# 115dkk/Impulcifer-pip313

Measured on AMD Instinct MI355X. Metric: impulse responses/sec (sweep deconv+FIR), 7.1×2-ear @48kHz, 1/2/4/8 GPU, higher is better.
Workload: dtype f32

## Files before the change

### impulcifer-pip313_amd/csrc/conv_kernels.hip.h

```cpp
#pragma once
#include "fft_regs.hip.h"

namespace imp {

constexpr int kN2 = 4096;
constexpr int kLogN2 = 12;
constexpr int kRowPad = 272;
#ifndef IMP_AB_PREFETCH
#define IMP_AB_PREFETCH 8
#endif
constexpr int kAbPrefetch = IMP_AB_PREFETCH;

struct Twiddles {
  const cf* __restrict__ full;
  const cf* __restrict__ hi;
  const cf* __restrict__ t1;
  const cf* __restrict__ t2;
  const cf* __restrict__ t4;
};

__device__ __forceinline__ void xcd_work_item(int nchan, int& tile, int& chan) {
  const int xcd = blockIdx.x & 7;
  const int slot = blockIdx.x >> 3;
  const int tl = slot / nchan;
// ... 818 lines not shown
#pragma unroll
  for (int j = 0; j < 16; ++j) bstore_cf<IMP_AUX_ROWS_ST>(v[j], r_row, vo8, j * 256 * 8);
}

struct FirBlockArgs {
  const float4* __restrict__ ab;
  long long ab_chan_stride;
  float* __restrict__ out;
  long long out_stride;
  long long out_start, out_len;
  int kp;
  int valid;
  int blocks;
  int first_block;
  int nchan;
};

constexpr int kFirBlockPoints = 4 * kN2;
constexpr size_t kFirBlockLds = sizeof(cf) * 4 * 16 * kRowPad;

template <class L, class = void> struct LoadHasDeviceLen { static constexpr bool value = false; };
template <class L> struct LoadHasDeviceLen<L, decltype((void)L::kDeviceLen)> { static constexpr bool value = true; };

template <class Load>
__global__ __launch_bounds__(1024, 4) void fir_block_kernel(Load ld, FirBlockArgs a, Twiddles tw) {
  extern __shared__ __attribute__((aligned(16))) char smem_raw[];
  cf* lds = reinterpret_cast<cf*>(smem_raw);
  const int xcd = blockIdx.x & 7, slot = blockIdx.x >> 3;
  const int chan = (slot / a.blocks) * 8 + xcd, blk = a.first_block + slot % a.blocks;
  if (chan >= a.nchan) return;
  long long out_len = a.out_len;
  int filt = chan;
  if constexpr (LoadHasDeviceLen<Load>::value) {
    out_len = ld.out_len(chan);
    filt = ld.filter_of(chan);
    if ((long long)blk * a.valid - a.out_start >= out_len) return;
  }
  const int tid = threadIdx.x;
  const int pairq = __builtin_amdgcn_readfirstlane(tid >> 9);
  const int half = __builtin_amdgcn_readfirstlane((tid >> 8) & 1);
  const int t = tid & 255;
  const int k1 = pairq + 2 * half;
  const int s0 = blk * a.valid - a.kp;
  const __amdgpu_buffer_rsrc_t r_full = make_rsrc(tw.full, 4u * kN2 * 8u);
  const auto row = ld.open(chan);

  cf v[16];
#pragma unroll
  for (int h = 0; h < 2; ++h) {
    cf x[2][4], w[2][3];
#pragma unroll
    for (int c = 0; c < 2; ++c) {
      const int n2 = tid + 1024 * (2 * h + c);
#pragma unroll
      for (int n1 = 0; n1 < 4; ++n1) x[c][n1] = row.pair_at(s0 + 2 * (n1 * kN2 + n2));
#pragma unroll
      for (int k = 1; k < 4; ++k) w[c][k - 1] = bload_cf(r_full, (unsigned)(k * kN2 + n2) * 8u, 0u);
    }
#pragma unroll
    for (int c = 0; c < 2; ++c) {
      const int n2 = tid + 1024 * (2 * h + c);
#pragma unroll
      for (int n1 = 0; n1 < 4; ++n1) x[c][n1] = row.finish(x[c][n1], s0 + 2 * (n1 * kN2 + n2));
      bfly4<-1>(x[c][0], x[c][1], x[c][2], x[c][3]);
      lds[n2] = x[c][0];
#pragma unroll
      for (int k = 1; k < 4; ++k) lds[k * kN2 + n2] = cmul(x[c][k], w[c][k - 1]);
    }
// ... 18 lines not shown
    cf w0 = lds[n2], w1 = lds[kN2 + n2], w2 = lds[2 * kN2 + n2], w3 = lds[3 * kN2 + n2];
    w1 = cmulc(w1, bload_cf(r_full, (unsigned)(kN2 + n2) * 8u, 0u));
    w2 = cmulc(w2, bload_cf(r_full, (unsigned)(2 * kN2 + n2) * 8u, 0u));
    w3 = cmulc(w3, bload_cf(r_full, (unsigned)(3 * kN2 + n2) * 8u, 0u));
    bfly4<+1>(w0, w1, w2, w3);
    const cf y[4] = {w0, w1, w2, w3};
#pragma unroll
    for (int n1 = 0; n1 < 4; ++n1) {
      const int pos = 2 * (n1 * kN2 + n2);
      if (pos < a.kp) continue;
      const unsigned off = (unsigned)(o0 + pos) * 4u;
      if (a.out_start & 1) {
        unsigned off_im = off + 4u;
        asm volatile("" : "+v"(off_im));
        __builtin_amdgcn_raw_buffer_store_b32(__float_as_uint(y[n1].x), r_out, off, 0u, 0);
        __builtin_amdgcn_raw_buffer_store_b32(__float_as_uint(y[n1].y), r_out, off_im, 0u, 0);
      } else {
        bstore_cf<kStreamAux>(y[n1], r_out, off, 0u);
      }
    }
  }
}

}
```

### impulcifer-pip313_amd/csrc/impulse_hip.hip

```cpp
#include <hip/hip_runtime.h>

#include <algorithm>
#include <cmath>
#include <complex>
#include <cstdarg>
#include <cstdio>
#include <cstdlib>
#include <cstring>
#include <map>
#include <mutex>
#include <new>
#include <string>
#include <vector>

#include "internal.h"
#include "conv_kernels.hip.h"
#include "ir_kernels.hip.h"
#include "decay_kernels.hip.h"
#include "slice_kernels.hip.h"

static thread_local std::string g_last_error;

int imp_fail(int code, const char* fmt, ...) {
  char buf[1024];
  va_list ap;
  va_start(ap, fmt);
  vsnprintf(buf, sizeof(buf), fmt, ap);
  va_end(ap);
  g_last_error = buf;
  return code;
}

int ctx_bind(imp_ctx* ctx) {
// ... 994 lines not shown
  if (!p->timing) return IMP_OK;
  if (slot == 0) p->group_timed = (p->group_counter++ % p->timing) == 0;
  if (!p->group_timed) return IMP_OK;
  if (p->timed >= kMaxTimed) {
    int rc = plan_collect_timing(p);
    if (rc) return rc;
  }
  const size_t need = (size_t)(4 * (p->timed + 1));
  while (p->events.size() < need) {
    hipEvent_t ev;
    HIP_TRY(hipEventCreate(&ev));
    p->events.push_back(ev);
  }
  HIP_TRY(hipEventRecord(p->events[(size_t)(4 * p->timed + slot)], p->cur_stream));
  if (slot == 3) ++p->timed;
  return IMP_OK;
}

template <class Load>
static int run_group_with(imp_plan* p, Load ld, int64_t nchan, float* d_y, int64_t chan_stride_out,
                          int64_t first_chan, int last_stage);

template <class Load>
static int launch_fir_block(imp_plan* p, Load ld, int64_t nchan, float* d_y, int64_t chan_stride_out, int64_t first_chan) {
  auto kern = imp::fir_block_kernel<Load>;
  int rc = ctx_kernel_lds(p->ctx, reinterpret_cast<const void*>(kern), imp::kFirBlockLds);
  if (rc) return rc;
  const int64_t plane = (int64_t)4 * imp::kN2;
  imp::FirBlockArgs a;
  a.ab = p->ab + (p->n_filters > 1 ? first_chan * plane : 0);
  a.ab_chan_stride = p->n_filters > 1 ? plane : 0;
  a.out = d_y;
  a.out_stride = chan_stride_out;
  a.out_start = p->out_start;
  a.first_block = (int)p->f_first;
  a.out_len = p->out_len;
  a.kp = p->f_kp;
  a.valid = p->f_valid;
  a.blocks = (int)p->f_blocks;
  a.nchan = (int)nchan;
  imp::Twiddles tw{p->tw.full, p->tw.hi, p->ctx->tw_t1, p->ctx->tw_t2, p->ctx->tw_t4};
  dim3 grid((unsigned)((nchan + 7) / 8 * 8 * p->f_blocks)), block(1024);
  hipLaunchKernelGGL(kern, grid, block, imp::kFirBlockLds, p->cur_stream, ld, a, tw);
  HIP_TRY(hipGetLastError());
  return IMP_OK;
}

template <class Load>
static int run_group_pair(imp_plan* p, Load ld, int64_t nchan, float* d_y, int64_t chan_stride_out, int last_stage) {
  int rc;
  const int64_t lane_channels = p->ws_channels / p->lanes;
  const int lane = (p->lanes > 1) ? (int)(p->group_counter_lane++ % p->lanes) : 0;
  p->cur_stream = lane ? p->ctx->side_streams[(size_t)(lane - 1)] : p->ctx->stream;
  p->cur_ws = p->ws + (int64_t)lane * (lane_channels / 2) * p->N1 * imp::kN2;
  if (nchan < 1 || nchan > lane_channels || (lane_channels & 1))
    return fail(IMP_ERR_INVALID, "launch group of %lld channels exceeds the workspace lane (%lld, whole pairs)",
                (long long)nchan, (long long)lane_channels);
  const int64_t npairs = (nchan + 1) / 2;
  if ((double)(chan_stride_out + p->out_len) * 4.0 >= 4294967296.0)
    return fail(IMP_ERR_INVALID, "chan_stride_out %lld: a pair's two output rows must lie within 4 GiB", (long long)chan_stride_out);
  imp::StoreWorkspace stw{p->cur_ws, p->N1};
  if ((rc = timing_event(p, 0))) return rc;
  if ((rc = launch_cols_any<-1>(p, npairs, ld, stw))) return rc;
  if ((rc = timing_event(p, 1))) return rc;
  if (last_stage < 1) return IMP_OK;
  if ((rc = launch_rows_single(p, npairs))) return rc;
  if ((rc = timing_event(p, 2))) return rc;
// ... 373 lines not shown
  return rc;
}

struct imp_chain {
  imp_ctx* ctx = nullptr;
  imp_ctx* tail_ctx = nullptr;
  imp_plan* deconv = nullptr;
  imp_plan* fir = nullptr;
  int64_t B = 0, n = 0, head = 0, fade_in = 0, fade_out = 0, pitch_ir = 0;
  double peak_height = 0.12589;
  int lanes = 1;
  int sets = 1;
  int64_t calls = 0;
  int tiles = 0;
  int64_t chunks = 0;
  std::vector<float*> d_ir;
  std::vector<unsigned*> d_tile;
  std::vector<imp::RowPeak*> d_res;
  std::vector<hipEvent_t> k1_done;
  std::vector<hipEvent_t> ir_free;
  std::vector<char> ir_busy;
  int64_t* d_meta = nullptr;
  double* d_win = nullptr;
};

struct ChainLock {
  std::unique_lock<std::recursive_mutex> a, b;
  ChainLock(imp_ctx* x, imp_ctx* y) {
    if (x == y) {
      a = std::unique_lock<std::recursive_mutex>(x->mu);
    } else {
      imp_ctx* lo = x < y ? x : y;
      imp_ctx* hi = x < y ? y : x;
      a = std::unique_lock<std::recursive_mutex>(lo->mu);
      b = std::unique_lock<std::recursive_mutex>(hi->mu);
    }
  }
};

extern "C" void imp_chain_destroy(imp_chain* c) {
  if (!c) return;
  ChainLock lk(c->ctx, c->tail_ctx);
  (void)hipSetDevice(c->ctx->device);
  (void)plan_sync_lanes(c->deconv);
  (void)hipStreamSynchronize(c->tail_ctx->stream);
  for (auto p : c->d_ir) (void)hipFree(p);
// ... 28 lines not shown
  if (fir->n_filters > 1 && B > fir->n_filters) return fail(IMP_ERR_INVALID, "imp_chain_create: fewer FIRs than channels");
  if (n > deconv->out_len || head < 0 || fade_in < 0 || fade_out < 0 || fade_in > n || fade_out > n)
    return fail(IMP_ERR_INVALID, "imp_chain_create: crop of %lld samples with fades %lld / %lld does not fit", (long long)n,
                (long long)fade_in, (long long)fade_out);
  if ((deconv->paired ? deconv->N1 / 2 : deconv->N1) > imp::kMaxPlanRows)
    return fail(IMP_ERR_UNSUPPORTED, "imp_chain_create: deconvolution plan of %d rows", deconv->N1);
  int rc = ctx_bind(deconv->ctx);
  if (rc) return rc;
  imp_chain* c = new (std::nothrow) imp_chain();
  if (!c) return fail(IMP_ERR_ALLOC, "out of host memory");
  c->ctx = deconv->ctx;
  c->tail_ctx = fir->ctx;
  c->deconv = deconv;
  c->fir = fir;
  c->B = B;
  c->n = n;
  c->head = head;
  c->fade_in = fade_in;
  c->fade_out = fade_out;
  c->peak_height = peak_height;
  c->lanes = deconv->lanes;
  c->sets = deconv->ctx == fir->ctx ? 1 : c->lanes + 1;
  c->pitch_ir = (deconv->out_len + 63) / 64 * 64;
  std::vector<int64_t> meta((size_t)(2 * B));
  for (int64_t b = 0; b < B; ++b) {
    meta[(size_t)b] = b * c->pitch_ir;
    meta[(size_t)(B + b)] = deconv->out_len;
  }
  c->tiles = plan_col_tiles(deconv);
  c->chunks = deconv->paired ? deconv->N1 / 2 : deconv->N1;
  const size_t chunk_bytes = (size_t)(B * c->chunks) * sizeof(unsigned);
  bool ok = hipMalloc((void**)&c->d_meta, (size_t)(2 * B) * sizeof(int64_t)) == hipSuccess &&
            hipMemcpy(c->d_meta, meta.data(), meta.size() * sizeof(int64_t), hipMemcpyHostToDevice) == hipSuccess &&
            hipMalloc((void**)&c->d_win, (size_t)std::max<int64_t>(fade_in + fade_out, 1) * sizeof(double)) == hipSuccess;
  if (ok && fade_in + fade_out > 0) {
    hipLaunchKernelGGL(imp::fade_table_kernel, dim3((unsigned)((fade_in + fade_out + 255) / 256)), dim3(256), 0, deconv->ctx->stream,
                       c->d_win, (long long)fade_in, (long long)fade_out);
    ok = hipGetLastError() == hipSuccess && hipStreamSynchronize(deconv->ctx->stream) == hipSuccess;
  }
  for (int l = 0; l < c->sets && ok; ++l) {
    float* ir = nullptr;
    unsigned* tile = nullptr;
    imp::RowPeak* res = nullptr;
    hipEvent_t e1 = nullptr, e2 = nullptr;
    ok = hipMalloc((void**)&ir, (size_t)(B * c->pitch_ir) * sizeof(float)) == hipSuccess;
    if (ir) c->d_ir.push_back(ir);
// ... 20 lines not shown
                                        float* d_out, int64_t chan_stride_out, long long* d_peaks_out) {
  if (!c || !d_x || !d_out) return fail(IMP_ERR_INVALID, "imp_chain_execute_device: null argument");
  ChainLock lk(c->ctx, c->tail_ctx);
  if (chan_stride_out < c->fir->out_len)
    return fail(IMP_ERR_INVALID, "chan_stride_out %lld < out_len %lld", (long long)chan_stride_out, (long long)c->fir->out_len);
  if (c->deconv->lanes != c->lanes || c->fir->lanes != 1)
    return fail(IMP_ERR_INVALID, "imp_chain_execute_device: a plan's overlap setting changed since the chain was made");
  int rc = ctx_bind(c->ctx);
  if (rc) return rc;
  const int lane = c->lanes > 1 ? (int)(c->deconv->group_counter_lane % c->lanes) : 0;
  const int l = (int)(c->calls++ % c->sets);
  hipStream_t lane_stream = lane ? c->ctx->side_streams[(size_t)(lane - 1)] : c->ctx->stream;
  hipStream_t tail = c->tail_ctx->stream;
  if (c->ir_busy[(size_t)l] && tail != lane_stream) HIP_TRY(hipStreamWaitEvent(lane_stream, c->ir_free[(size_t)l], 0));
  c->deconv->tile_max = c->d_tile[(size_t)l];
  rc = imp_conv_execute_device(c->deconv, d_x, c->B, chan_stride_in, elem_stride_in, c->d_ir[(size_t)l], c->pitch_ir);
  c->deconv->tile_max = nullptr;
  if (rc) return rc;
  if (c->deconv->cur_stream != lane_stream) return fail(IMP_ERR_HIP, "imp_chain_execute_device: lane bookkeeping out of step");
  if (tail != lane_stream) {
    HIP_TRY(hipEventRecord(c->k1_done[(size_t)l], lane_stream));
    HIP_TRY(hipStreamWaitEvent(tail, c->k1_done[(size_t)l], 0));
  }
  hipLaunchKernelGGL(imp::row_first_peak_chunked_kernel, dim3((unsigned)c->B), dim3(imp::kPeakThreads), 0, tail, c->d_ir[(size_t)l],
                     c->d_meta, c->d_meta + c->B, c->deconv->out_start, (const unsigned*)c->d_tile[(size_t)l], c->tiles,
                     (const unsigned*)nullptr, c->chunks, c->d_res[(size_t)l], c->peak_height, d_peaks_out);
  HIP_TRY(hipGetLastError());
  imp::LoadCropAtPeak ld{c->d_ir[(size_t)l], c->pitch_ir, c->deconv->out_len, c->d_res[(size_t)l], c->n, c->head, c->fade_in, c->fade_out,
                         c->d_win};
  if ((rc = run_group_with(c->fir, ld, c->B, d_out, chan_stride_out, 0, 2))) return rc;
  if (tail != lane_stream) {
    HIP_TRY(hipEventRecord(c->ir_free[(size_t)l], tail));
    c->ir_busy[(size_t)l] = 1;
  }
  return IMP_OK;
}

struct imp_segset {
  imp_ctx* ctx = nullptr;
  int64_t B = 0;
  double* e = nullptr;
  int64_t* off = nullptr;
  int64_t* len = nullptr;
  std::vector<int64_t> h_len;
  void* qbuf = nullptr;
  size_t qcap = 0;
  void* keep_a = nullptr;
  void* keep_b = nullptr;
  std::vector<int64_t> keep_host;
};

extern "C" void imp_segset_destroy(imp_segset* s) {
  if (!s) return;
// ... 667 lines not shown
```

### impulcifer-pip313_amd/csrc/ir_kernels.hip.h

```cpp
#pragma once
#include <hip/hip_runtime.h>
#include <stdint.h>

#include "conv_kernels.hip.h"

namespace imp {

struct RowPeak {
  unsigned int maxabs_bits;
  unsigned int pad;
  unsigned long long first_peak;
  unsigned long long first_max;
};

constexpr int kPeakChunk = 8192;
#ifdef IMP_PEAK_DIAG
#define IMP_PEAK_T(k) do { if (threadIdx.x == 0 && blockIdx.x == 0) peak_ts[k] = clock64(); } while (0)
#else
#define IMP_PEAK_T(k) do { } while (0)
#endif
constexpr int kPeakThreads = 1024;
constexpr int kMaxPlanRows = 256;

__device__ __forceinline__ int64_t peak_chunks(int64_t n, int64_t shift) {
// ... 7 lines not shown
  __syncthreads();
  if ((threadIdx.x & 63) == 0) wm[threadIdx.x >> 6] = m;
  __syncthreads();
  float r = wm[0];
#pragma unroll
  for (int k = 1; k < NW; ++k) r = fmaxf(r, wm[k]);
  return r;
}

template <int NW>
__device__ __forceinline__ unsigned long long block_min_u64(unsigned long long v, unsigned long long* wm ) {
#pragma unroll
  for (int s = 32; s > 0; s >>= 1) {
    const unsigned long long o = __shfl_xor(v, s, 64);
    v = o < v ? o : v;
  }
  __syncthreads();
  if ((threadIdx.x & 63) == 0) wm[threadIdx.x >> 6] = v;
  __syncthreads();
  unsigned long long r = wm[0];
#pragma unroll
  for (int k = 1; k < NW; ++k) r = wm[k] < r ? wm[k] : r;
  return r;
}

__global__ __launch_bounds__(256) void row_chunk_max_kernel(const float* __restrict__ x, const int64_t* __restrict__ off,
                                                            const int64_t* __restrict__ len, int64_t shift,
                                                            unsigned* __restrict__ chunk_max, int64_t pitch) {
  const int b = blockIdx.y;
  const int64_t n = len[b], c = blockIdx.x;
  if (c >= peak_chunks(n, shift)) return;
  const int64_t lo = c * kPeakChunk - shift > 0 ? c * kPeakChunk - shift : 0;
  const int64_t hi = (c + 1) * kPeakChunk - shift < n ? (c + 1) * kPeakChunk - shift : n;
  const float* row = x + off[b];
  float m = 0.f;
  int64_t i = lo + threadIdx.x;
  for (; i + 7 * 256 < hi; i += 8 * 256) {
    float v[8];
#pragma unroll
    for (int k = 0; k < 8; ++k) v[k] = row[i + k * 256];
#pragma unroll
    for (int k = 0; k < 8; ++k) m = fmaxf(m, fabsf(v[k]));
  }
  for (; i < hi; i += 256) m = fmaxf(m, fabsf(row[i]));
  __shared__ __attribute__((aligned(16))) float wm[4];
  m = block_max_f32<4>(m, wm);
  if (threadIdx.x == 0) chunk_max[(int64_t)b * pitch + c] = __float_as_uint(m);
}

__global__ __launch_bounds__(kPeakThreads) void row_first_peak_chunked_kernel(
    const float* __restrict__ x, const int64_t* __restrict__ off, const int64_t* __restrict__ len, int64_t shift,
    const unsigned* __restrict__ tile_max, int tiles, const unsigned* __restrict__ chunk_max, int64_t pitch,
    RowPeak* __restrict__ res, double height, long long* __restrict__ peaks_out) {
  const int b = blockIdx.x, tid = threadIdx.x;
#ifdef IMP_PEAK_DIAG
  long long peak_ts[8] = {0, 0, 0, 0, 0, 0, 0, 0};
#endif
  IMP_PEAK_T(0);
  const int64_t n = len[b];
  const float* row = x + off[b];
  const int64_t nch = peak_chunks(n, shift);
  constexpr int NW = kPeakThreads / 64;
  __shared__ __attribute__((aligned(16))) float wmf[NW];
  __shared__ __attribute__((aligned(16))) unsigned long long wmu[NW];
  __shared__ float sx[kPeakChunk + 2];
  constexpr int kLdsChunks = 2048;
  __shared__ unsigned srows[kLdsChunks];
  const unsigned* cm = chunk_max + (int64_t)b * pitch;
  if (tiles > 0) {
    for (int r = tid; r < kMaxPlanRows; r += kPeakThreads) srows[r] = 0u;
    __syncthreads();
    const unsigned* tm = tile_max + (int64_t)b * tiles * pitch;
    const int lane = tid & 63, w = tid >> 6;
    for (int64_t r = lane; r < nch; r += 64) {
      unsigned m = 0u;
#pragma unroll 4
      for (int t = w; t < tiles; t += kPeakThreads / 64) {
        const unsigned v = tm[(int64_t)t * pitch + r];
        m = v > m ? v : m;
      }
      if (m) atomicMax(&srows[r], m);
    }
    __syncthreads();
    cm = srows;
  } else if (nch <= kLdsChunks) {
    for (int64_t c = tid; c < nch; c += kPeakThreads) srows[c] = cm[c];
    __syncthreads();
    cm = srows;
  }
  IMP_PEAK_T(1);
  float mf = 0.f;
  for (int64_t c = tid; c < nch; c += kPeakThreads) mf = fmaxf(mf, __uint_as_float(cm[c]));
  const float maxabs = block_max_f32<NW>(mf, wmf);
  RowPeak out;
  out.maxabs_bits = __float_as_uint(maxabs);
  out.pad = 0u;
  out.first_peak = ~0ull;
  out.first_max = ~0ull;
  if (maxabs >= 1e-20f) {
    __shared__ float s_thr;
    if (tid == 0) {
      const double dmax = (double)maxabs;
      float t = (float)(height * dmax);
      if (!(t >= 0.f)) t = 0.f;
      for (int k = 0; k < 4 && t > 0.f && (double)__uint_as_float(__float_as_uint(t) - 1u) / dmax >= height; ++k)
        t = __uint_as_float(__float_as_uint(t) - 1u);
      for (int k = 0; k < 4 && !((double)t / dmax >= height); ++k) t = __uint_as_float(__float_as_uint(t) + 1u);
      s_thr = t;
    }
    __syncthreads();
    const float thr = s_thr;
    IMP_PEAK_T(2);
    unsigned long long c_q = ~0ull;
    for (int64_t c = tid; c < nch; c += kPeakThreads)
      if (__uint_as_float(cm[c]) >= thr && (unsigned long long)c < c_q) c_q = (unsigned long long)c;
    c_q = block_min_u64<NW>(c_q, wmu);
    constexpr int U = (kPeakChunk + kPeakThreads - 1) / kPeakThreads;
    int64_t lo = 0, hi = 0;
    auto stage = [&](int64_t c) {
      lo = c * kPeakChunk - shift > 0 ? c * kPeakChunk - shift : 0;
      hi = (c + 1) * kPeakChunk - shift < n ? (c + 1) * kPeakChunk - shift : n;
      const int64_t cnt = hi - lo + 2;
      float t[U + 1];
#pragma unroll
      for (int u = 0; u <= U; ++u) {
        const int64_t k = tid + (int64_t)u * kPeakThreads, i = lo - 1 + k;
        t[u] = (k < cnt && i >= 0 && i < n) ? row[i] : 0.f;
      }
      __syncthreads();
#pragma unroll
      for (int u = 0; u <= U; ++u) {
        const int64_t k = tid + (int64_t)u * kPeakThreads;
        if (k < cnt) sx[k] = t[u];
      }
      __syncthreads();
    };
    IMP_PEAK_T(3);
    for (int64_t c = c_q == ~0ull ? nch : (int64_t)c_q; c < nch; ++c) {
      if (!(__uint_as_float(cm[c]) >= thr)) continue;
      stage(c);
      IMP_PEAK_T(4);
      float xs[U];
#pragma unroll
      for (int u = 0; u < U; ++u) {
        const int64_t i = lo + tid + (int64_t)u * kPeakThreads;
        xs[u] = i < hi ? sx[i - lo + 1] : 0.f;
      }
      unsigned long long best = ~0ull;
#pragma unroll
      for (int u = 0; u < U; ++u) {
        const int64_t i = lo + tid + (int64_t)u * kPeakThreads;
        const float xi = xs[u];
        if (best != ~0ull || !(fabsf(xi) >= thr) || i >= hi || i == 0 || i >= n - 1) continue;
        const float xm = sx[i - lo];
        const bool up = xm < xi, dn = xm > xi;
        if (!up && !dn) continue;
        if (!((up ? xi : -xi) >= thr)) continue;
        int64_t j = i;
        while (j + 1 < n && (j + 1 <= hi ? sx[j + 1 - lo + 1] : row[j + 1]) == xi) ++j;
        if (j + 1 >= n) continue;
        const float xn = j + 1 <= hi ? sx[j + 1 - lo + 1] : row[j + 1];
        if (up ? (xn < xi) : (xn > xi)) best = (unsigned long long)((i + j) / 2);
      }
      best = block_min_u64<NW>(best, wmu);
      if (best != ~0ull) {
        out.first_peak = best;
        break;
      }
    }
    IMP_PEAK_T(5);
    if (out.first_peak == ~0ull) {
      unsigned long long c_max = ~0ull;
      for (int64_t c = tid; c < nch; c += kPeakThreads)
        if (__uint_as_float(cm[c]) == maxabs && (unsigned long long)c < c_max) c_max = (unsigned long long)c;
      c_max = block_min_u64<NW>(c_max, wmu);
      stage((int64_t)c_max);
      unsigned long long best = ~0ull;
      for (int64_t i = lo + tid; i < hi; i += kPeakThreads)
        if (fabsf(sx[i - lo + 1]) == maxabs) {
          best = (unsigned long long)i;
          break;
        }
      out.first_max = block_min_u64<NW>(best, wmu);
    }
  }
  IMP_PEAK_T(6);
#ifdef IMP_PEAK_DIAG
  if (tid == 0 && b == 0)
    printf("peak phases (clk): entry->fold %lld, max+thr %lld, cq %lld, stage %lld, search %lld, fallback %lld\n", peak_ts[1] - peak_ts[0],
           peak_ts[2] - peak_ts[1], peak_ts[3] - peak_ts[2], peak_ts[4] - peak_ts[3], peak_ts[5] - peak_ts[4], peak_ts[6] - peak_ts[5]);
#endif
  if (tid == 0) {
    res[b] = out;
    if (peaks_out) {
      long long pk;
      if (n == 0 || !(maxabs >= 1e-20f)) pk = 0;
      else pk = (long long)(out.first_peak != ~0ull ? out.first_peak : out.first_max);
      peaks_out[b] = pk;
    }
  }
}

__device__ __forceinline__ double hann_sym_fwd(int64_t i, int64_t N) {
  if (N <= 1) return 1.0;
  return 0.5 - 0.5 * cospi(2.0 * (double)i / (double)(N - 1));
}


__device__ __forceinline__ unsigned* crop_max_lds() {
  __shared__ unsigned rows[kMaxPlanRows];
  return rows;
}

struct StoreRealCropMax {
  StoreRealCrop crop;
  unsigned* __restrict__ tile_max;
  __device__ __forceinline__ __amdgpu_buffer_rsrc_t bind(int b) const { return crop.bind(b); }
  __device__ __forceinline__ void begin(int tid, int threads) const {
    unsigned* rows = crop_max_lds();
    for (int r = tid; r < kMaxPlanRows; r += threads) rows[r] = 0u;
    __syncthreads();
  }
// ... 61 lines not shown
    for (int r = tid; r < chunks; r += threads) out[r] = rl[r];
    if (2 * p + 1 < crop.nchan) {
      out += (long long)tiles * chunks;
      for (int r = tid; r < chunks; r += threads) out[r] = rr[r];
    }
  }
};

struct LoadCropAtPeak {
  const float* __restrict__ base;
  long long chan_stride;
  long long row_len;
  const RowPeak* __restrict__ res;
  long long n, head, fade_in, fade_out;
  const double* __restrict__ win;
  __host__ __device__ LoadCropAtPeak shifted(long long, long long) const { return *this; }
  static __device__ __forceinline__ float shaped(float x, long long i, long long n, long long fade_in, long long fade_out,
                                                 const double* __restrict__ win) {
    double g = 1.0;
    if (i < fade_in) g *= win[i];
    if (fade_out > 0 && i >= n - fade_out && i < n) g *= win[fade_in + (i - (n - fade_out))];
    return (float)((double)x * g);
  }
  __device__ __forceinline__ long long crop_start(int b) const {
    const RowPeak rp = res[b];
    long long pk;
    if (row_len == 0 || !(__uint_as_float(rp.maxabs_bits) >= 1e-20f)) pk = 0;
    else pk = (long long)(rp.first_peak != ~0ull ? rp.first_peak : rp.first_max);
    long long start = pk - head;
    if (start > row_len - n) start = row_len - n;
    if (start < 0) start = 0;
    return start;
  }
  struct Row {
    __amdgpu_buffer_rsrc_t r;
    int n, fade_in, fade_out;
    const double* __restrict__ win;
    __device__ __forceinline__ cf pair_at(int s) const { return bload_cf<0>(r, (unsigned)s * 4u, 0u); }
    __device__ __forceinline__ cf finish(cf v, int s) const {
      if ((unsigned)s < (unsigned)n && (s < fade_in || s + 1 >= n - fade_out)) {
        v.x = shaped(v.x, s, n, fade_in, fade_out, win);
        v.y = shaped(v.y, s + 1, n, fade_in, fade_out, win);
      }
      return v;
    }
  };
  __device__ __forceinline__ Row open(int b) const {
    const long long start = crop_start(b), avail = row_len - start;
    return Row{make_rsrc(base + (long long)b * chan_stride + start, (unsigned)(avail < n ? avail : n) * 4u), (int)n, (int)fade_in,
               (int)fade_out, win};
  }
  template <int STEP, int F>
  __device__ __forceinline__ void column(int b, unsigned e0, cf (&v)[F]) const {
    const long long start = crop_start(b), avail = row_len - start;
    const __amdgpu_buffer_rsrc_t r = make_rsrc(base + (long long)b * chan_stride + start, (unsigned)(avail < n ? avail : n) * 4u);
#pragma unroll
    for (int j = 0; j < F; ++j) {
      const u32x2 x = __builtin_amdgcn_raw_buffer_load_b64(r, e0 * 8u, (unsigned)(j * STEP) * 8u, 0);
      v[j] = make_float2(__uint_as_float(x.x), __uint_as_float(x.y));
      const long long i = 2ll * ((long long)e0 + (long long)j * STEP);
      if (i < n && (i < fade_in || i + 1 >= n - fade_out)) {
        v[j].x = shaped(v[j].x, i, n, fade_in, fade_out, win);
        v[j].y = shaped(v[j].y, i + 1, n, fade_in, fade_out, win);
      }
    }
  }
};

__global__ __launch_bounds__(256) void fade_table_kernel(double* __restrict__ win, long long fade_in, long long fade_out) {
  const long long i = (long long)blockIdx.x * blockDim.x + threadIdx.x;
  if (i < fade_in) win[i] = hann_sym_fwd(i, 2 * fade_in);
  else if (i < fade_in + fade_out) win[i] = hann_sym_fwd(fade_out + (i - fade_in), 2 * fade_out);
}

struct WindowParams {
  float gain;
  int64_t fade_in;
  int64_t fade_out;
  int64_t decay_start;
  int64_t decay_half;
  int64_t decay_knee;
  float decay_level_db;
};

__device__ __forceinline__ double hann_sym(int64_t i, int64_t N) {
  if (N <= 1) return 1.0;
  return 0.5 - 0.5 * cospi(2.0 * (double)i / (double)(N - 1));
}
// ... 565 lines not shown
```

Baseline: 299,400.

## Fold first-peak search into FIR block kernel and add 512-thread pairs variant

The separate row_first_peak_chunked_kernel launch is removed from the chain tail. Each FIR block kernel now runs the peak search itself in LDS before opening its cropped row, and the first block of each channel publishes the result. An optional 512-thread pairs kernel, selected by environment variable, processes the transform planes in two passes to raise occupancy. The peak search also uses wave-level reductions and a ballot-based threshold. The trade-off is that every block of a channel repeats the peak search, which adds per-block work and extra barriers in exchange for one fewer launch and one fewer serialization point.

```diff
diff --git a/impulcifer-pip313_amd/csrc/conv_kernels.hip.h b/impulcifer-pip313_amd/csrc/conv_kernels.hip.h
--- a/impulcifer-pip313_amd/csrc/conv_kernels.hip.h
+++ b/impulcifer-pip313_amd/csrc/conv_kernels.hip.h
@@ -864,6 +864,22 @@
 template <class L, class = void> struct LoadHasDeviceLen { static constexpr bool value = false; };
 template <class L> struct LoadHasDeviceLen<L, decltype((void)L::kDeviceLen)> { static constexpr bool value = true; };
 
+template <class L, class = void> struct LoadFindsPeak { static constexpr bool value = false; };
+template <class L> struct LoadFindsPeak<L, decltype((void)L::kFindsPeak)> { static constexpr bool value = true; };
+
+template <int NT, class Load>
+__device__ __forceinline__ auto open_block_row(const Load& ld, int chan, bool publish, char* lds) {
+  if constexpr (LoadFindsPeak<Load>::value) {
+    const auto rp = ld.template find<NT>(chan, lds);
+    if (threadIdx.x == 0 && publish) ld.publish(chan, rp);
+    const auto row = ld.open_at(chan, rp);
+    __syncthreads();
+    return row;
+  } else {
+    return ld.open(chan);
+  }
+}
+
 template <class Load>
 __global__ __launch_bounds__(1024, 4) void fir_block_kernel(Load ld, FirBlockArgs a, Twiddles tw) {
   extern __shared__ __attribute__((aligned(16))) char smem_raw[];
@@ -885,7 +901,7 @@
   const int k1 = pairq + 2 * half;
   const int s0 = blk * a.valid - a.kp;
   const __amdgpu_buffer_rsrc_t r_full = make_rsrc(tw.full, 4u * kN2 * 8u);
-  const auto row = ld.open(chan);
+  const auto row = open_block_row<1024>(ld, chan, slot % a.blocks == 0, smem_raw);
 
   cf v[16];
 #pragma unroll
@@ -950,4 +966,116 @@
   }
 }
 
-}
+
+constexpr int kFirPairsThreads = 512;
+constexpr size_t kFirPairsLds = sizeof(cf) * 2 * 16 * kRowPad;
+static_assert(sizeof(cf) * 2 * kN2 <= kFirPairsLds, "two rows of a block fit the planes");
+
+template <class Load>
+__global__ __launch_bounds__(kFirPairsThreads, 3) void fir_block_pairs_kernel(Load ld, FirBlockArgs a, Twiddles tw) {
+  extern __shared__ __attribute__((aligned(16))) char smem_raw[];
+  cf* lds = reinterpret_cast<cf*>(smem_raw);
+  constexpr int NT = kFirPairsThreads, C = kN2 / NT;
+  const int xcd = blockIdx.x & 7, slot = blockIdx.x >> 3;
+  const int chan = (slot / a.blocks) * 8 + xcd, blk = a.first_block + slot % a.blocks;
+  if (chan >= a.nchan) return;
+  const int tid = threadIdx.x;
+  const int half = __builtin_amdgcn_readfirstlane(tid >> 8);
+  const int t = tid & 255;
+  const int s0 = blk * a.valid - a.kp;
+  const __amdgpu_buffer_rsrc_t r_full = make_rsrc(tw.full, 4u * kN2 * 8u);
+
+  const auto row = open_block_row<NT>(ld, chan, slot % a.blocks == 0, smem_raw);
+
+  cf park[2 * C];
+#pragma unroll
+  for (int h = 0; h < C / 2; ++h) {
+    cf x[2][4], w[2][3];
+#pragma unroll
+    for (int c = 0; c < 2; ++c) {
+      const int n2 = tid + NT * (2 * h + c);
+#pragma unroll
+      for (int n1 = 0; n1 < 4; ++n1) x[c][n1] = row.pair_at(s0 + 2 * (n1 * kN2 + n2));
+#pragma unroll
+      for (int k = 1; k < 4; ++k) w[c][k - 1] = bload_cf(r_full, (unsigned)(k * kN2 + n2) * 8u, 0u);
+    }
+#pragma unroll
+    for (int c = 0; c < 2; ++c) {
+      const int n2 = tid + NT * (2 * h + c), cc = 2 * h + c;
+#pragma unroll
+      for (int n1 = 0; n1 < 4; ++n1) x[c][n1] = row.finish(x[c][n1], s0 + 2 * (n1 * kN2 + n2));
+      bfly4<-1>(x[c][0], x[c][1], x[c][2], x[c][3]);
+      lds[n2] = x[c][0];
+      lds[kN2 + n2] = cmul(x[c][2], w[c][1]);
+      park[cc] = cmul(x[c][1], w[c][0]);
+      park[C + cc] = cmul(x[c][3], w[c][2]);
+    }
+  }
+  const __amdgpu_buffer_rsrc_t r_ab0 = make_rsrc(a.ab + (long long)chan * a.ab_chan_stride + (long long)(2 * half) * kN2,
+                                                 kN2 * sizeof(float4));
+  const __amdgpu_buffer_rsrc_t r_ab1 = make_rsrc(a.ab + (long long)chan * a.ab_chan_stride + (long long)(1 + 2 * half) * kN2,
+                                                 kN2 * sizeof(float4));
+  cf v[16];
+  __syncthreads();
+#pragma unroll
+  for (int j = 0; j < 16; ++j) v[j] = lds[half * kN2 + t + 256 * j];
+  __syncthreads();
+  rows_core<0, 1>(v, lds, half, 0, 2 * half, r_ab0, tw, t);
+  __syncthreads();
+#pragma unroll
+  for (int cc = 0; cc < C; ++cc) {
+    const int n2 = tid + NT * cc;
+    lds[n2] = park[cc];
+    lds[kN2 + n2] = park[C + cc];
+  }
+#pragma unroll
+  for (int j = 0; j < 16; ++j) park[j] = v[j];
+  __syncthreads();
+#pragma unroll
+  for (int j = 0; j < 16; ++j) v[j] = lds[half * kN2 + t + 256 * j];
+  __syncthreads();
+  rows_core<0, 1>(v, lds, half, 1, 1 + 2 * half, r_ab1, tw, t);
+
+  __syncthreads();
+#pragma unroll
+  for (int j = 0; j < 16; ++j) lds[half * kN2 + t + 256 * j] = v[j];
+  __syncthreads();
+#pragma unroll
+  for (int cc = 0; cc < C; ++cc) {
+    const int n2 = tid + NT * cc;
+    v[cc] = lds[n2];
+    v[C + cc] = lds[kN2 + n2];
+  }
+  __syncthreads();
+#pragma unroll
+  for (int j = 0; j < 16; ++j) lds[half * kN2 + t + 256 * j] = park[j];
+  __syncthreads();
+  const __amdgpu_buffer_rsrc_t r_out = make_rsrc(a.out + (long long)chan * a.out_stride, (unsigned)a.out_len * 4u);
+  const int o0 = blk * a.valid - a.kp - (int)a.out_start;
+#pragma unroll
+  for (int cc = 0; cc < C; ++cc) {
+    const int n2 = tid + NT * cc;
+    cf w0 = lds[n2], w1 = v[cc], w2 = lds[kN2 + n2], w3 = v[C + cc];
+    w1 = cmulc(w1, bload_cf(r_full, (unsigned)(kN2 + n2) * 8u, 0u));
+    w2 = cmulc(w2, bload_cf(r_full, (unsigned)(2 * kN2 + n2) * 8u, 0u));
+    w3 = cmulc(w3, bload_cf(r_full, (unsigned)(3 * kN2 + n2) * 8u, 0u));
+    bfly4<+1>(w0, w1, w2, w3);
+    const cf y[4] = {w0, w1, w2, w3};
+#pragma unroll
+    for (int n1 = 0; n1 < 4; ++n1) {
+      const int pos = 2 * (n1 * kN2 + n2);
+      if (pos < a.kp) continue;
+      const unsigned off = (unsigned)(o0 + pos) * 4u;
+      if (a.out_start & 1) {
+        unsigned off_im = off + 4u;
+        asm volatile("" : "+v"(off_im));
+        __builtin_amdgcn_raw_buffer_store_b32(__float_as_uint(y[n1].x), r_out, off, 0u, 0);
+        __builtin_amdgcn_raw_buffer_store_b32(__float_as_uint(y[n1].y), r_out, off_im, 0u, 0);
+      } else {
+        bstore_cf<kStreamAux>(y[n1], r_out, off, 0u);
+      }
+    }
+  }
+}
+
+}
diff --git a/impulcifer-pip313_amd/csrc/impulse_hip.hip b/impulcifer-pip313_amd/csrc/impulse_hip.hip
--- a/impulcifer-pip313_amd/csrc/impulse_hip.hip
+++ b/impulcifer-pip313_amd/csrc/impulse_hip.hip
@@ -9,6 +9,7 @@
 #include <cstring>
 #include <map>
 #include <mutex>
+#include <type_traits>
 #include <new>
 #include <string>
 #include <vector>
@@ -1049,9 +1050,13 @@
                           int64_t first_chan, int last_stage);
 
 template <class Load>
-static int launch_fir_block(imp_plan* p, Load ld, int64_t nchan, float* d_y, int64_t chan_stride_out, int64_t first_chan) {
-  auto kern = imp::fir_block_kernel<Load>;
-  int rc = ctx_kernel_lds(p->ctx, reinterpret_cast<const void*>(kern), imp::kFirBlockLds);
+static int launch_fir_block(imp_plan* p, Load ld, int64_t nchan, float* d_y, int64_t chan_stride_out, int64_t first_chan,
+                            bool pairs = false) {
+  const void* kern = reinterpret_cast<const void*>(imp::fir_block_kernel<Load>);
+  if constexpr (std::is_same<Load, imp::LoadFindPeak>::value)
+    if (pairs) kern = reinterpret_cast<const void*>(imp::fir_block_pairs_kernel<Load>);
+  const size_t lds = pairs ? imp::kFirPairsLds : imp::kFirBlockLds;
+  int rc = ctx_kernel_lds(p->ctx, kern, lds);
   if (rc) return rc;
   const int64_t plane = (int64_t)4 * imp::kN2;
   imp::FirBlockArgs a;
@@ -1067,9 +1072,33 @@
   a.blocks = (int)p->f_blocks;
   a.nchan = (int)nchan;
   imp::Twiddles tw{p->tw.full, p->tw.hi, p->ctx->tw_t1, p->ctx->tw_t2, p->ctx->tw_t4};
-  dim3 grid((unsigned)((nchan + 7) / 8 * 8 * p->f_blocks)), block(1024);
-  hipLaunchKernelGGL(kern, grid, block, imp::kFirBlockLds, p->cur_stream, ld, a, tw);
+  dim3 grid((unsigned)((nchan + 7) / 8 * 8 * p->f_blocks));
+  if constexpr (std::is_same<Load, imp::LoadFindPeak>::value) {
+    if (pairs) {
+      hipLaunchKernelGGL(imp::fir_block_pairs_kernel<Load>, grid, dim3(imp::kFirPairsThreads), lds, p->cur_stream, ld, a, tw);
+      HIP_TRY(hipGetLastError());
+      return IMP_OK;
+    }
+  }
+  hipLaunchKernelGGL(imp::fir_block_kernel<Load>, grid, dim3(1024), lds, p->cur_stream, ld, a, tw);
   HIP_TRY(hipGetLastError());
+  return IMP_OK;
+}
+
+static int run_chain_tail(imp_plan* p, const imp::LoadFindPeak& ld, int64_t nchan, float* d_y, int64_t chan_stride_out, bool pairs) {
+  int rc;
+  p->cur_stream = p->ctx->stream;
+  p->cur_ws = p->ws;
+  if (!p->fused || p->lanes != 1 || p->paired || p->tile_max) return fail(IMP_ERR_INVALID, "run_chain_tail: not a fused FIR plan of one lane");
+  if (nchan < 1 || nchan > p->ws_channels)
+    return fail(IMP_ERR_INVALID, "launch group of %lld channels exceeds the workspace (%lld)", (long long)nchan, (long long)p->ws_channels);
+  if (p->n_filters > 1 && nchan > p->n_filters)
+    return fail(IMP_ERR_INVALID, "channel %lld has no filter: the plan holds %lld per-channel filters", (long long)(nchan - 1),
+                (long long)p->n_filters);
+  if ((rc = timing_event(p, 0))) return rc;
+  if ((rc = launch_fir_block(p, ld, nchan, d_y, chan_stride_out, 0, pairs))) return rc;
+  for (int slot = 1; slot <= 3; ++slot)
+    if ((rc = timing_event(p, slot))) return rc;
   return IMP_OK;
 }
 
@@ -1489,6 +1518,7 @@
   std::vector<char> ir_busy;
   int64_t* d_meta = nullptr;
   double* d_win = nullptr;
+  enum Tail { kTailLegacy, kTailFolded, kTailPairs } tail_mode = kTailLegacy;
 };
 
 struct ChainLock {
@@ -1563,6 +1593,9 @@
   c->lanes = deconv->lanes;
   c->sets = deconv->ctx == fir->ctx ? 1 : c->lanes + 1;
   c->pitch_ir = (deconv->out_len + 63) / 64 * 64;
+  const char* tail_env = std::getenv("IMPULSE_HIP_CHAIN_TAIL");
+  if (fir->fused && !(tail_env && std::strcmp(tail_env, "legacy") == 0))
+    c->tail_mode = tail_env && std::strcmp(tail_env, "pairs") == 0 ? imp_chain::kTailPairs : imp_chain::kTailFolded;
   std::vector<int64_t> meta((size_t)(2 * B));
   for (int64_t b = 0; b < B; ++b) {
     meta[(size_t)b] = b * c->pitch_ir;
@@ -1629,13 +1662,19 @@
     HIP_TRY(hipEventRecord(c->k1_done[(size_t)l], lane_stream));
     HIP_TRY(hipStreamWaitEvent(tail, c->k1_done[(size_t)l], 0));
   }
-  hipLaunchKernelGGL(imp::row_first_peak_chunked_kernel, dim3((unsigned)c->B), dim3(imp::kPeakThreads), 0, tail, c->d_ir[(size_t)l],
-                     c->d_meta, c->d_meta + c->B, c->deconv->out_start, (const unsigned*)c->d_tile[(size_t)l], c->tiles,
-                     (const unsigned*)nullptr, c->chunks, c->d_res[(size_t)l], c->peak_height, d_peaks_out);
-  HIP_TRY(hipGetLastError());
   imp::LoadCropAtPeak ld{c->d_ir[(size_t)l], c->pitch_ir, c->deconv->out_len, c->d_res[(size_t)l], c->n, c->head, c->fade_in, c->fade_out,
                          c->d_win};
-  if ((rc = run_group_with(c->fir, ld, c->B, d_out, chan_stride_out, 0, 2))) return rc;
+  if (c->tail_mode != imp_chain::kTailLegacy) {
+    const imp::LoadFindPeak lf{ld, (const unsigned*)c->d_tile[(size_t)l], c->tiles, c->chunks, c->deconv->out_start, c->peak_height,
+                               c->d_res[(size_t)l], d_peaks_out};
+    if ((rc = run_chain_tail(c->fir, lf, c->B, d_out, chan_stride_out, c->tail_mode == imp_chain::kTailPairs))) return rc;
+  } else {
+    hipLaunchKernelGGL(imp::row_first_peak_chunked_kernel, dim3((unsigned)c->B), dim3(imp::kPeakThreads), 0, tail, c->d_ir[(size_t)l],
+                       c->d_meta, c->d_meta + c->B, c->deconv->out_start, (const unsigned*)c->d_tile[(size_t)l], c->tiles,
+                       (const unsigned*)nullptr, c->chunks, c->d_res[(size_t)l], c->peak_height, d_peaks_out);
+    HIP_TRY(hipGetLastError());
+    if ((rc = run_group_with(c->fir, ld, c->B, d_out, chan_stride_out, 0, 2))) return rc;
+  }
   if (tail != lane_stream) {
     HIP_TRY(hipEventRecord(c->ir_free[(size_t)l], tail));
     c->ir_busy[(size_t)l] = 1;
diff --git a/impulcifer-pip313_amd/csrc/ir_kernels.hip.h b/impulcifer-pip313_amd/csrc/ir_kernels.hip.h
--- a/impulcifer-pip313_amd/csrc/ir_kernels.hip.h
+++ b/impulcifer-pip313_amd/csrc/ir_kernels.hip.h
@@ -53,6 +53,21 @@
 #pragma unroll
   for (int k = 1; k < NW; ++k) r = wm[k] < r ? wm[k] : r;
   return r;
+}
+
+__device__ __forceinline__ float wave_max_f32(float m) {
+#pragma unroll
+  for (int s = 32; s > 0; s >>= 1) m = fmaxf(m, __shfl_xor(m, s, 64));
+  return m;
+}
+
+__device__ __forceinline__ unsigned long long wave_min_u64(unsigned long long v) {
+#pragma unroll
+  for (int s = 32; s > 0; s >>= 1) {
+    const unsigned long long o = __shfl_xor(v, s, 64);
+    v = o < v ? o : v;
+  }
+  return v;
 }
 
 __global__ __launch_bounds__(256) void row_chunk_max_kernel(const float* __restrict__ x, const int64_t* __restrict__ off,
@@ -79,34 +94,36 @@
   if (threadIdx.x == 0) chunk_max[(int64_t)b * pitch + c] = __float_as_uint(m);
 }
 
-__global__ __launch_bounds__(kPeakThreads) void row_first_peak_chunked_kernel(
-    const float* __restrict__ x, const int64_t* __restrict__ off, const int64_t* __restrict__ len, int64_t shift,
-    const unsigned* __restrict__ tile_max, int tiles, const unsigned* __restrict__ chunk_max, int64_t pitch,
-    RowPeak* __restrict__ res, double height, long long* __restrict__ peaks_out) {
-  const int b = blockIdx.x, tid = threadIdx.x;
+struct PeakLds {
+  float* sx;
+  unsigned* srows;
+  float* wmf;
+  unsigned long long* wmu;
+};
+constexpr int kLdsChunks = 2048;
+constexpr size_t kPeakLdsBytes = sizeof(float) * (kPeakChunk + 2 + 2) + sizeof(unsigned) * kLdsChunks + 16 * (4 + 8);
+
+template <int NT>
+__device__ __forceinline__ RowPeak first_peak_search(const float* __restrict__ row, const int64_t n, const int64_t shift,
+                                                     const unsigned* __restrict__ tm, const int tiles, const unsigned* cm,
+                                                     const int64_t pitch, const double height, const PeakLds s) {
+  const int tid = threadIdx.x;
 #ifdef IMP_PEAK_DIAG
   long long peak_ts[8] = {0, 0, 0, 0, 0, 0, 0, 0};
 #endif
   IMP_PEAK_T(0);
-  const int64_t n = len[b];
-  const float* row = x + off[b];
   const int64_t nch = peak_chunks(n, shift);
-  constexpr int NW = kPeakThreads / 64;
-  __shared__ __attribute__((aligned(16))) float wmf[NW];
-  __shared__ __attribute__((aligned(16))) unsigned long long wmu[NW];
-  __shared__ float sx[kPeakChunk + 2];
-  constexpr int kLdsChunks = 2048;
-  __shared__ unsigned srows[kLdsChunks];
-  const unsigned* cm = chunk_max + (int64_t)b * pitch;
+  constexpr int NW = NT / 64;
+  float* sx = s.sx;
+  unsigned* srows = s.srows;
   if (tiles > 0) {
-    for (int r = tid; r < kMaxPlanRows; r += kPeakThreads) srows[r] = 0u;
-    __syncthreads();
-    const unsigned* tm = tile_max + (int64_t)b * tiles * pitch;
+    for (int r = tid; r < kMaxPlanRows; r += NT) srows[r] = 0u;
+    __syncthreads();
     const int lane = tid & 63, w = tid >> 6;
     for (int64_t r = lane; r < nch; r += 64) {
       unsigned m = 0u;
 #pragma unroll 4
-      for (int t = w; t < tiles; t += kPeakThreads / 64) {
+      for (int t = w; t < tiles; t += NW) {
         const unsigned v = tm[(int64_t)t * pitch + r];
         m = v > m ? v : m;
       }
@@ -115,38 +132,51 @@
     __syncthreads();
     cm = srows;
   } else if (nch <= kLdsChunks) {
-    for (int64_t c = tid; c < nch; c += kPeakThreads) srows[c] = cm[c];
+    for (int64_t c = tid; c < nch; c += NT) srows[c] = cm[c];
     __syncthreads();
     cm = srows;
   }
   IMP_PEAK_T(1);
-  float mf = 0.f;
-  for (int64_t c = tid; c < nch; c += kPeakThreads) mf = fmaxf(mf, __uint_as_float(cm[c]));
-  const float maxabs = block_max_f32<NW>(mf, wmf);
+  const bool cm_lds = cm == srows;
+  const int lane = tid & 63;
+  float maxabs;
+  if (cm_lds) {
+    float mf = 0.f;
+    for (int64_t c = lane; c < nch; c += 64) mf = fmaxf(mf, __uint_as_float(cm[c]));
+    maxabs = wave_max_f32(mf);
+  } else {
+    float mf = 0.f;
+    for (int64_t c = tid; c < nch; c += NT) mf = fmaxf(mf, __uint_as_float(cm[c]));
+    maxabs = block_max_f32<NW>(mf, s.wmf);
+  }
   RowPeak out;
   out.maxabs_bits = __float_as_uint(maxabs);
   out.pad = 0u;
   out.first_peak = ~0ull;
   out.first_max = ~0ull;
   if (maxabs >= 1e-20f) {
-    __shared__ float s_thr;
-    if (tid == 0) {
-      const double dmax = (double)maxabs;
-      float t = (float)(height * dmax);
-      if (!(t >= 0.f)) t = 0.f;
-      for (int k = 0; k < 4 && t > 0.f && (double)__uint_as_float(__float_as_uint(t) - 1u) / dmax >= height; ++k)
-        t = __uint_as_float(__float_as_uint(t) - 1u);
-      for (int k = 0; k < 4 && !((double)t / dmax >= height); ++k) t = __uint_as_float(__float_as_uint(t) + 1u);
-      s_thr = t;
-    }
-    __syncthreads();
-    const float thr = s_thr;
+    const double dmax = (double)maxabs;
+    float t0 = (float)(height * dmax);
+    if (!(t0 >= 0.f)) t0 = 0.f;
+    const unsigned b0 = __float_as_uint(t0);
+    const bool pass_l = lane < 9 && (double)__uint_as_float(b0 + (unsigned)(lane - 4)) / dmax >= height;
+    const unsigned long long pass = __ballot(pass_l);
+    int o = 0;
+    for (int k = 0; k < 4 && __uint_as_float(b0 + (unsigned)o) > 0.f && ((pass >> (4 + o - 1)) & 1ull); ++k) --o;
+    for (int k = 0; k < 4 && !((pass >> (4 + o)) & 1ull); ++k) ++o;
+    const float thr = __uint_as_float(b0 + (unsigned)o);
     IMP_PEAK_T(2);
     unsigned long long c_q = ~0ull;
-    for (int64_t c = tid; c < nch; c += kPeakThreads)
-      if (__uint_as_float(cm[c]) >= thr && (unsigned long long)c < c_q) c_q = (unsigned long long)c;
-    c_q = block_min_u64<NW>(c_q, wmu);
-    constexpr int U = (kPeakChunk + kPeakThreads - 1) / kPeakThreads;
+    if (cm_lds) {
+      for (int64_t c = lane; c < nch; c += 64)
+        if (__uint_as_float(cm[c]) >= thr && (unsigned long long)c < c_q) c_q = (unsigned long long)c;
+      c_q = wave_min_u64(c_q);
+    } else {
+      for (int64_t c = tid; c < nch; c += NT)
+        if (__uint_as_float(cm[c]) >= thr && (unsigned long long)c < c_q) c_q = (unsigned long long)c;
+      c_q = block_min_u64<NW>(c_q, s.wmu);
+    }
+    constexpr int U = (kPeakChunk + NT - 1) / NT;
     int64_t lo = 0, hi = 0;
     auto stage = [&](int64_t c) {
       lo = c * kPeakChunk - shift > 0 ? c * kPeakChunk - shift : 0;
@@ -155,13 +185,13 @@
       float t[U + 1];
 #pragma unroll
       for (int u = 0; u <= U; ++u) {
-        const int64_t k = tid + (int64_t)u * kPeakThreads, i = lo - 1 + k;
+        const int64_t k = tid + (int64_t)u * NT, i = lo - 1 + k;
         t[u] = (k < cnt && i >= 0 && i < n) ? row[i] : 0.f;
       }
       __syncthreads();
 #pragma unroll
       for (int u = 0; u <= U; ++u) {
-        const int64_t k = tid + (int64_t)u * kPeakThreads;
+        const int64_t k = tid + (int64_t)u * NT;
         if (k < cnt) sx[k] = t[u];
       }
       __syncthreads();
@@ -174,13 +204,13 @@
       float xs[U];
 #pragma unroll
       for (int u = 0; u < U; ++u) {
-        const int64_t i = lo + tid + (int64_t)u * kPeakThreads;
+        const int64_t i = lo + tid + (int64_t)u * NT;
         xs[u] = i < hi ? sx[i - lo + 1] : 0.f;
       }
       unsigned long long best = ~0ull;
 #pragma unroll
       for (int u = 0; u < U; ++u) {
-        const int64_t i = lo + tid + (int64_t)u * kPeakThreads;
+        const int64_t i = lo + tid + (int64_t)u * NT;
         const float xi = xs[u];
         if (best != ~0ull || !(fabsf(xi) >= thr) || i >= hi || i == 0 || i >= n - 1) continue;
         const float xm = sx[i - lo];
@@ -193,7 +223,7 @@
         const float xn = j + 1 <= hi ? sx[j + 1 - lo + 1] : row[j + 1];
         if (up ? (xn < xi) : (xn > xi)) best = (unsigned long long)((i + j) / 2);
       }
-      best = block_min_u64<NW>(best, wmu);
+      best = block_min_u64<NW>(best, s.wmu);
       if (best != ~0ull) {
         out.first_peak = best;
         break;
@@ -202,33 +232,49 @@
     IMP_PEAK_T(5);
     if (out.first_peak == ~0ull) {
       unsigned long long c_max = ~0ull;
-      for (int64_t c = tid; c < nch; c += kPeakThreads)
+      for (int64_t c = tid; c < nch; c += NT)
         if (__uint_as_float(cm[c]) == maxabs && (unsigned long long)c < c_max) c_max = (unsigned long long)c;
-      c_max = block_min_u64<NW>(c_max, wmu);
+      c_max = block_min_u64<NW>(c_max, s.wmu);
       stage((int64_t)c_max);
       unsigned long long best = ~0ull;
-      for (int64_t i = lo + tid; i < hi; i += kPeakThreads)
+      for (int64_t i = lo + tid; i < hi; i += NT)
         if (fabsf(sx[i - lo + 1]) == maxabs) {
           best = (unsigned long long)i;
           break;
         }
-      out.first_max = block_min_u64<NW>(best, wmu);
+      out.first_max = block_min_u64<NW>(best, s.wmu);
     }
   }
   IMP_PEAK_T(6);
 #ifdef IMP_PEAK_DIAG
-  if (tid == 0 && b == 0)
+  if (tid == 0 && blockIdx.x == 0)
     printf("peak phases (clk): entry->fold %lld, max+thr %lld, cq %lld, stage %lld, search %lld, fallback %lld\n", peak_ts[1] - peak_ts[0],
            peak_ts[2] - peak_ts[1], peak_ts[3] - peak_ts[2], peak_ts[4] - peak_ts[3], peak_ts[5] - peak_ts[4], peak_ts[6] - peak_ts[5]);
 #endif
-  if (tid == 0) {
+  return out;
+}
+
+__device__ __forceinline__ long long peak_index_of(const RowPeak& rp, long long n) {
+  if (n == 0 || !(__uint_as_float(rp.maxabs_bits) >= 1e-20f)) return 0;
+  return (long long)(rp.first_peak != ~0ull ? rp.first_peak : rp.first_max);
+}
+
+__global__ __launch_bounds__(kPeakThreads) void row_first_peak_chunked_kernel(
+    const float* __restrict__ x, const int64_t* __restrict__ off, const int64_t* __restrict__ len, int64_t shift,
+    const unsigned* __restrict__ tile_max, int tiles, const unsigned* __restrict__ chunk_max, int64_t pitch,
+    RowPeak* __restrict__ res, double height, long long* __restrict__ peaks_out) {
+  const int b = blockIdx.x;
+  const int64_t n = len[b];
+  __shared__ __attribute__((aligned(16))) float wmf[kPeakThreads / 64];
+  __shared__ __attribute__((aligned(16))) unsigned long long wmu[kPeakThreads / 64];
+  __shared__ float sx[kPeakChunk + 2];
+  __shared__ unsigned srows[kLdsChunks];
+  const RowPeak out = first_peak_search<kPeakThreads>(x + off[b], n, shift, tile_max + (int64_t)b * tiles * pitch, tiles,
+                                                      chunk_max + (int64_t)b * pitch, pitch, height,
+                                                      PeakLds{sx, srows, wmf, wmu});
+  if (threadIdx.x == 0) {
     res[b] = out;
-    if (peaks_out) {
-      long long pk;
-      if (n == 0 || !(maxabs >= 1e-20f)) pk = 0;
-      else pk = (long long)(out.first_peak != ~0ull ? out.first_peak : out.first_max);
-      peaks_out[b] = pk;
-    }
+    if (peaks_out) peaks_out[b] = peak_index_of(out, n);
   }
 }
 
@@ -336,16 +382,13 @@
     if (fade_out > 0 && i >= n - fade_out && i < n) g *= win[fade_in + (i - (n - fade_out))];
     return (float)((double)x * g);
   }
-  __device__ __forceinline__ long long crop_start(int b) const {
-    const RowPeak rp = res[b];
-    long long pk;
-    if (row_len == 0 || !(__uint_as_float(rp.maxabs_bits) >= 1e-20f)) pk = 0;
-    else pk = (long long)(rp.first_peak != ~0ull ? rp.first_peak : rp.first_max);
-    long long start = pk - head;
+  __device__ __forceinline__ long long crop_start_at(const RowPeak& rp) const {
+    long long start = peak_index_of(rp, row_len) - head;
     if (start > row_len - n) start = row_len - n;
     if (start < 0) start = 0;
     return start;
   }
+  __device__ __forceinline__ long long crop_start(int b) const { return crop_start_at(res[b]); }
   struct Row {
     __amdgpu_buffer_rsrc_t r;
     int n, fade_in, fade_out;
@@ -359,8 +402,9 @@
       return v;
     }
   };
-  __device__ __forceinline__ Row open(int b) const {
-    const long long start = crop_start(b), avail = row_len - start;
+  __device__ __forceinline__ Row open(int b) const { return open_at(b, crop_start(b)); }
+  __device__ __forceinline__ Row open_at(int b, long long start) const {
+    const long long avail = row_len - start;
     return Row{make_rsrc(base + (long long)b * chan_stride + start, (unsigned)(avail < n ? avail : n) * 4u), (int)n, (int)fade_in,
                (int)fade_out, win};
   }
@@ -378,6 +422,37 @@
         v[j].y = shaped(v[j].y, i + 1, n, fade_in, fade_out, win);
       }
     }
+  }
+};
+
+struct LoadFindPeak {
+  LoadCropAtPeak crop;
+  const unsigned* __restrict__ tile_max;
+  int tiles;
+  long long pitch, shift;
+  double height;
+  RowPeak* __restrict__ res;
+  long long* __restrict__ peaks_out;
+  using Row = LoadCropAtPeak::Row;
+  static constexpr bool kFindsPeak = true;
+  template <int NT>
+  __device__ __forceinline__ RowPeak find(int b, char* lds) const {
+    constexpr size_t o_rows = (sizeof(float) * (kPeakChunk + 2) + 15) / 16 * 16, o_wmf = o_rows + sizeof(unsigned) * kLdsChunks,
+                     o_wmu = o_wmf + sizeof(float) * 16, o_end = o_wmu + sizeof(unsigned long long) * 16;
+    static_assert(NT <= 1024 && o_end <= kPeakLdsBytes, "PeakLds layout");
+    const PeakLds s{reinterpret_cast<float*>(lds), reinterpret_cast<unsigned*>(lds + o_rows), reinterpret_cast<float*>(lds + o_wmf),
+                    reinterpret_cast<unsigned long long*>(lds + o_wmu)};
+    return first_peak_search<NT>(crop.base + (long long)b * crop.chan_stride, crop.row_len, shift,
+                                 tile_max + (long long)b * tiles * pitch, tiles, nullptr, pitch, height, s);
+  }
+  __device__ __forceinline__ void publish(int b, const RowPeak& rp) const {
+    res[b] = rp;
+    if (peaks_out) peaks_out[b] = peak_index_of(rp, crop.row_len);
+  }
+  __device__ __forceinline__ Row open_at(int b, const RowPeak& rp) const {
+    const unsigned long long st = (unsigned long long)crop.crop_start_at(rp);
+    const unsigned lo = __builtin_amdgcn_readfirstlane((unsigned)st), hi = __builtin_amdgcn_readfirstlane((unsigned)(st >> 32));
+    return crop.open_at(b, (long long)(((unsigned long long)hi << 32) | lo));
   }
 };
 
```

New measurement: 305,000 (median of 6 runs). 1.02x the previous value.
